# simonsobs/Pixell.jl

Hardware: AMD Instinct MI355X
Metric: Mpix/s CAR bilinear reproject (Float64) + % HBM roofline, 1/2/4/8 MI355X (higher is better)
Workload: dtype f64

## Files before the change

pixell.jl_amd/csrc/pxl_kernels.hip:

```cpp
#include <hip/hip_runtime.h>

#include <algorithm>
#include <mutex>
#include <vector>
#include <cmath>
#include <cstdarg>
#include <cstdio>
#include <cstring>
#include <new>
#include <type_traits>

#include "pxl_device.h"

using namespace pxl;

static thread_local char g_err[512] = "";

static int fail(int code, const char* fmt, ...) {
    va_list ap;
    va_start(ap, fmt);
    vsnprintf(g_err, sizeof(g_err), fmt, ap);
    va_end(ap);
    return code;
}
// ... 1131 lines not shown
int pxl_reproject_execute_f32(pxl_reproject_plan* pl, const float* src, float* dst, void* stream) {
    int rc = pxl_reproject_build_tables(pl, stream);
    if (rc) return rc;
    return pxl_reproject_execute_rows_f32(pl, src, dst, 0, pl->dst_nrows, stream);
}

int pxl_reproject_plan_src_rows(const pxl_reproject_plan* pl, int64_t* lo, int64_t* hi) {
    if (!pl || !lo || !hi) return fail(PXL_EINVAL, "plan_src_rows: null argument");
    int64_t l = INT64_MAX, h = INT64_MIN;
    for (int64_t r = 0; r < pl->dst_nrows; ++r) {
        int64_t j0 = pl->h_yj0[pl->dst_row0 + r];
        for (int64_t j = j0; j <= j0 + 1; ++j)
            if (j >= 1 && j <= pl->ny) { if (j - 1 < l) l = j - 1; if (j > h) h = j; }
    }
    if (l > h) { l = 0; h = 0; }
    *lo = l; *hi = h;
    return PXL_OK;
}

int pxl_reproject_plan_rows_covered(const pxl_reproject_plan* pl, int64_t have_lo, int64_t have_hi, int64_t* lo,
                                    int64_t* hi) {
    if (!pl || !lo || !hi) return fail(PXL_EINVAL, "plan_rows_covered: null argument");
    int64_t best_lo = 0, best_hi = 0, cur_lo = -1;
    for (int64_t r = 0; r <= pl->dst_nrows; ++r) {
        bool ok = false;
        if (r < pl->dst_nrows) {
            int64_t j0 = pl->h_yj0[pl->dst_row0 + r];
            ok = true;
            for (int64_t j = j0; j <= j0 + 1; ++j)
                if (j >= 1 && j <= pl->ny && !(j - 1 >= have_lo && j - 1 < have_hi)) ok = false;
        }
        if (ok) { if (cur_lo < 0) cur_lo = r; }
        else if (cur_lo >= 0) {
            if (r - cur_lo > best_hi - best_lo) { best_lo = cur_lo; best_hi = r; }
            cur_lo = -1;
        }
    }
    *lo = best_lo; *hi = best_hi;
    return PXL_OK;
}

int pxl_comm_unique_id(void* id128) {
    if (!id128) return fail(PXL_EINVAL, "comm_unique_id: null buffer (PXL_COMM_ID_BYTES bytes)");
    const RcclApi& nc = rccl_api(true);
    if (!nc.ok) return fail(PXL_ENODEV, "comm_unique_id: RCCL not available: %s", nc.where);
    static_assert(sizeof(ncclUniqueId) == PXL_COMM_ID_BYTES, "ncclUniqueId size");
    ncclUniqueId id;
    ncclResult_t r = nc.GetUniqueId(&id);
    if (r != ncclSuccess) return fail(PXL_EHIP, "comm_unique_id: ncclGetUniqueId: %s", nc.GetErrorString(r));
    memcpy(id128, &id, sizeof id);
    return PXL_OK;
}

int pxl_comm_init_rank(const void* id128, int rank, int nranks, void** comm) {
    if (!id128 || !comm) return fail(PXL_EINVAL, "comm_init_rank: null argument");
    *comm = nullptr;
    if (nranks < 1 || rank < 0 || rank >= nranks) return fail(PXL_EINVAL, "comm_init_rank: rank %d outside [0, %d)", rank, nranks);
    const RcclApi& nc = rccl_api(true);
    if (!nc.ok) return fail(PXL_ENODEV, "comm_init_rank: RCCL not available: %s", nc.where);
    ncclUniqueId id;
    memcpy(&id, id128, sizeof id);
    ncclComm_t c = nullptr;
    ncclResult_t r = nc.CommInitRank(&c, nranks, id, rank);
    if (r != ncclSuccess) return fail(PXL_EHIP, "comm_init_rank: ncclCommInitRank: %s", nc.GetErrorString(r));
    rccl_own_comm_add((void*)c);
    *comm = (void*)c;
    return PXL_OK;
}

int pxl_comm_destroy(void* comm) {
    if (!comm) return PXL_OK;
    if (!rccl_own_comm_erase(comm)) return fail(PXL_EINVAL, "comm_destroy: not a communicator created by pxl_comm_init_rank");
    const RcclApi& nc = rccl_api(false);
    if (!nc.ok) return fail(PXL_ENODEV, "comm_destroy: RCCL not available: %s", nc.where);
    ncclResult_t r = nc.CommDestroy((ncclComm_t)comm);
    if (r != ncclSuccess) return fail(PXL_EHIP, "comm_destroy: ncclCommDestroy: %s", nc.GetErrorString(r));
    return PXL_OK;
}

const char* pxl_comm_backend(void) {
    static thread_local char where[256];
    const RcclApi nc = rccl_api(false);
    snprintf(where, sizeof where, "%s", nc.where);
    return where;
}

int pxl_reproject_sharded_step_f64(pxl_reproject_plan* plan, double* src, double* dst, int64_t own_row0, int64_t own_nrows,
                                   const pxl_halo_xfer* sends, int nsends, const pxl_halo_xfer* recvs, int nrecvs,
                                   void* rccl_comm, void* stream) {
    return sharded_step_impl(plan, src, dst, own_row0, own_nrows, sends, nsends, recvs, nrecvs, rccl_comm, stream);
}

int pxl_reproject_sharded_step_f32(pxl_reproject_plan* plan, float* src, float* dst, int64_t own_row0, int64_t own_nrows,
                                   const pxl_halo_xfer* sends, int nsends, const pxl_halo_xfer* recvs, int nrecvs,
                                   void* rccl_comm, void* stream) {
    return sharded_step_impl(plan, src, dst, own_row0, own_nrows, sends, nsends, recvs, nrecvs, rccl_comm, stream);
}

int pxl_reproject_car_bilinear_f64(const pxl_car_wcs* wcs_in, const int64_t shape_in[3], const double* src,
                                   const pxl_car_wcs* wcs_out, const int64_t shape_out[2], double* dst,
                                   void* stream) {
    if (!shape_in || !shape_out) return fail(PXL_EINVAL, "reproject: null shape");
    pxl_reproject_plan* pl = nullptr;
    int rc = pxl_reproject_plan_create(wcs_in, shape_in, 0, shape_in[1], wcs_out, shape_out, 0, shape_out[1], &pl);
    if (rc) return rc;
    rc = pxl_reproject_execute(pl, src, dst, stream);
    if (rc == PXL_OK) {
        hipError_t e = hipStreamSynchronize((hipStream_t)stream);
        if (e != hipSuccess) rc = fail(PXL_EHIP, "reproject: %s", hipGetErrorString(e));
    }
    pxl_reproject_plan_destroy(pl);
    return rc;
}

int pxl_reproject_generic_last_tiles(int64_t* exact_tiles, int64_t* total_tiles, void* stream) {
    if (!exact_tiles || !total_tiles) return fail(PXL_EINVAL, "generic_last_tiles: null argument");
    int64_t total = 0;
    unsigned int* c = last_exact_word(-1, &total);
    if (!c) return fail(PXL_ENODEV, "generic_last_tiles: no counter on this device");
    unsigned int v = 0;
    HIP_TRY(hipMemcpyAsync(&v, c, 4, hipMemcpyDeviceToHost, (hipStream_t)stream));
    HIP_TRY(hipStreamSynchronize((hipStream_t)stream));
    *exact_tiles = v; *total_tiles = total;
    return PXL_OK;
}

struct pxl_generic_plan {
    GenericParams p;
    int64_t gx, gy, ntiles, exact;
    char* mem;
    LatticeWs ws;
    int device;
};

int pxl_generic_plan_create(const pxl_car_wcs* wcs_in, int proj_in, const int64_t shape_in[2],
                            const pxl_car_wcs* wcs_out, int proj_out, const int64_t shape_out[2],
                            void* stream, pxl_generic_plan** plan) {
    if (!plan) return fail(PXL_EINVAL, "generic_plan_create: null result");
    *plan = nullptr;
    GenericParams p;
    int rc = generic_params("generic_plan_create", wcs_in, proj_in, shape_in, wcs_out, proj_out, shape_out, &p);
    if (rc) return rc;
    const int64_t gx = (p.nxo + PXL_TW - 1) / PXL_TW, gy = (p.nyo + PXL_TH - 1) / PXL_TH;
    if (gy > 65535) return fail(PXL_EINVAL, "generic_plan_create: more than 65 535 tile rows (use the one-shot entry)");
    const int64_t ntiles = gx * gy;
    pxl_generic_plan* pl = new (std::nothrow) pxl_generic_plan();
    if (!pl) return fail(PXL_ENOMEM, "generic_plan_create: out of host memory");
    hipStream_t st = (hipStream_t)stream;
    hipError_t e = hipGetDevice(&pl->device);
    if (e == hipSuccess) e = hipMalloc((void**)&pl->mem, lattice_layout(nullptr, ntiles).bytes);
    if (e != hipSuccess) { (void)hipGetLastError(); delete pl; return fail(PXL_EHIP, "generic_plan_create: %s", hipGetErrorString(e)); }
    pl->ws = lattice_layout(pl->mem, ntiles);
    pl->gx = gx; pl->gy = gy; pl->ntiles = ntiles;
    p.exact_tiles = pl->ws.counter; p.exact_tiles_last = nullptr;
    pl->p = p;
    unsigned int host_count = 0;
    e = lattice_build(p, gx, ntiles, pl->ws, st);
    if (e == hipSuccess) e = hipGetLastError();
    if (e == hipSuccess) e = hipMemcpyAsync(&host_count, pl->ws.counter, 4, hipMemcpyDeviceToHost, st);
    if (e == hipSuccess) e = hipStreamSynchronize(st);
    if (e != hipSuccess) { (void)hipFree(pl->mem); delete pl; return fail(PXL_EHIP, "generic_plan_create: %s", hipGetErrorString(e)); }
    pl->exact = host_count;
    *plan = pl;
    return PXL_OK;
}

int pxl_generic_plan_execute(const pxl_generic_plan* plan, int64_t ncomp, const double* src, double* dst, void* stream) {
    if (!plan) return fail(PXL_EINVAL, "generic_plan_execute: null plan");
    if (ncomp < 1 || ncomp > 0x7fffffff) return fail(PXL_EINVAL, "generic_plan_execute: component count must be positive");
    if (!src || !dst) return fail(PXL_EINVAL, "generic_plan_execute: null src/dst");
    int dev = -1;
    if (hipGetDevice(&dev) != hipSuccess || dev != plan->device) return fail(PXL_EINVAL, "generic_plan_execute: plan belongs to device %d, current device is %d", plan->device, dev);
    GenericParams p = plan->p;
    p.src = src; p.dst = dst; p.nc = (int32_t)ncomp;
    hipStream_t st = (hipStream_t)stream;
    hipLaunchKernelGGL(k_reproject_generic_tiled3, dim3((unsigned)plan->gx, (unsigned)plan->gy), dim3(256), 0, st, p, (const double2*)plan->ws.lat, (const int32_t*)plan->ws.flag);
    if (plan->exact > 0)
        hipLaunchKernelGGL(k_reproject_generic_exact_tiles, dim3((unsigned)std::min<int64_t>(plan->ntiles, 256)), dim3(256), 0, st, p, (const int32_t*)plan->ws.flag, plan->gx, plan->ntiles);
    return check_launch("k_reproject_generic_tiled3 (plan)");
}

int pxl_generic_plan_tiles(const pxl_generic_plan* plan, int64_t* exact_tiles, int64_t* total_tiles) {
    if (!plan || !exact_tiles || !total_tiles) return fail(PXL_EINVAL, "generic_plan_tiles: null argument");
    *exact_tiles = plan->exact; *total_tiles = plan->ntiles;
    return PXL_OK;
}

int pxl_generic_plan_destroy(pxl_generic_plan* plan) {
    if (!plan) return PXL_OK;
    hipError_t e = plan->mem ? hipFree(plan->mem) : hipSuccess;
    delete plan;
    if (e != hipSuccess) return fail(PXL_EHIP, "generic_plan_destroy: %s", hipGetErrorString(e));
    return PXL_OK;
}

int pxl_reproject_generic_bilinear_f64(const pxl_car_wcs* wcs_in, int proj_in, const int64_t shape_in[3],
                                       const double* src, const pxl_car_wcs* wcs_out, int proj_out,
                                       const int64_t shape_out[2], double* dst, void* stream) {
    GenericParams p;
    int rcp = generic_params("reproject_generic", wcs_in, proj_in, shape_in, wcs_out, proj_out, shape_out, &p);
    if (rcp) return rcp;
    if (shape_in[2] < 1) return fail(PXL_EINVAL, "reproject_generic: shapes must be positive");
    if (!src || !dst) return fail(PXL_EINVAL, "reproject_generic: null src/dst");
    p.src = src; p.dst = dst; p.nc = (int32_t)shape_in[2];
    const int64_t gx = (p.nxo + PXL_TW - 1) / PXL_TW, gy = (p.nyo + PXL_TH - 1) / PXL_TH;
    if (env_int("PXL_GENERIC_EXACT", 0) || gy > 65535) {
        hipLaunchKernelGGL(k_reproject_generic, dim3(stream_grid(p.nxo * p.nyo, 256)), dim3(256), 0, (hipStream_t)stream, p);
        return check_launch("k_reproject_generic");
    }
    const int64_t ntiles = gx * gy;
    p.exact_tiles_last = last_exact_word(ntiles);
    hipStream_t st = (hipStream_t)stream;
    Scratch mem;
    if (int rc = mem.alloc(lattice_layout(nullptr, ntiles).bytes, st)) return rc;
    const LatticeWs ws = lattice_layout(mem.p, ntiles);
    p.exact_tiles = ws.counter;
    hipError_t me = lattice_build(p, gx, ntiles, ws, st);
    if (me != hipSuccess) {
        (void)hipGetLastError();
        return fail(PXL_EHIP, "reproject_generic: hipMemsetAsync: %s", hipGetErrorString(me));
    }
    hipLaunchKernelGGL(k_reproject_generic_tiled3, dim3((unsigned)gx, (unsigned)gy), dim3(256), 0, st, p, (const double2*)ws.lat, (const int32_t*)ws.flag);
    hipLaunchKernelGGL(k_reproject_generic_exact_tiles, dim3((unsigned)std::min<int64_t>(ntiles, 256)), dim3(256), 0, st, p, (const int32_t*)ws.flag, gx, ntiles);
    return mem.release("reproject_generic", check_launch("k_reproject_generic_tiled3"));
}

int pxl_sample_car_bilinear_f64(const pxl_car_wcs* wcs_in, const int64_t shape_in[3], const double* src,
                                int64_t src_row0, int64_t src_nrows, int64_t n, const double* sky, double* out,
                                void* stream) {
    return sample_impl(wcs_in, shape_in, src, src_row0, src_nrows, n, sky, out, stream);
}

int pxl_scatter_car_bilinear_f64(const pxl_car_wcs* wcs, const int64_t shape[3], double* dst, int64_t row0, int64_t nrows,
                                 int64_t n, const double* sky, const double* vals, void* stream) {
    PointCall c("scatter", wcs, shape, n, sky);
    if (int rc = check_points(c.rows(row0, nrows).reads(vals, 0).writes(dst, 0))) return rc;
    return launch_points(c, "k_scatter_bilinear", k_scatter_bilinear, PXL_SUNR, stream, dst, shape[0], shape[1], (int32_t)shape[2], row0, nrows,
                         car_periodic(wcs, shape[0]), n, (const double2*)sky, vals);
}

int pxl_sample_car_bilinear_f32(const pxl_car_wcs* wcs_in, const int64_t shape_in[3], const float* src,
                                int64_t src_row0, int64_t src_nrows, int64_t n, const double* sky, float* out,
                                void* stream) {
    return sample_impl(wcs_in, shape_in, src, src_row0, src_nrows, n, sky, out, stream);
}

int pxl_spline_prefilter_car_f64(const pxl_car_wcs* wcs, const int64_t shape[3], const double* src, double* coeffs, void* stream) {
    return spline_prefilter_impl<false>("spline_prefilter", wcs, shape, src, coeffs, stream);
}

int pxl_spline_prefilter_transpose_car_f64(const pxl_car_wcs* wcs, const int64_t shape[3], const double* src, double* dst, void* stream) {
    return spline_prefilter_impl<true>("spline_prefilter_transpose", wcs, shape, src, dst, stream);
}

int pxl_reproject_car_cubic_f64(const pxl_car_wcs* wcs_in, const int64_t shape_in[3], const double* coeffs,
                                const pxl_car_wcs* wcs_out, const int64_t shape_out[2], double* dst, void* stream) {
    if (!wcs_ok(wcs_in) || !wcs_ok(wcs_out)) return fail(PXL_EINVAL, "reproject_cubic: invalid WCS");
    if (int rc = spline_shape_check("reproject_cubic", shape_in)) return rc;
    if (!shape_out || shape_out[0] < 1 || shape_out[1] < 1) return fail(PXL_EINVAL, "reproject_cubic: output shape must be positive");
    if (shape_out[0] > 1000000000 || shape_out[1] > 65535LL * PXL_SPL_TH) return fail(PXL_EINVAL, "reproject_cubic: output axis too long");
    if (!coeffs || !dst) return fail(PXL_EINVAL, "reproject_cubic: null coefficients or output");
    const int64_t nx = shape_in[0], ny = shape_in[1], nc = shape_in[2], nxo = shape_out[0], nyo = shape_out[1];
    const uintptr_t cb = (uintptr_t)nx * (uintptr_t)ny * (uintptr_t)nc * 8, db = (uintptr_t)nxo * (uintptr_t)nyo * (uintptr_t)nc * 8;
    if (overlaps(coeffs, cb, dst, db)) return fail(PXL_EINVAL, "reproject_cubic: dst overlaps coeffs");
    hipStream_t st = (hipStream_t)stream;
    Scratch mem;
    if (int rc = mem.alloc(table_layout(nullptr, nxo, nyo).bytes, st)) return rc;
    const Tables t = table_layout(mem.p, nxo, nyo);
    SplineReproj p;
    p.coeffs = coeffs; p.dst = dst;
    p.xfx = t.xfx; p.yfy = t.yfy; p.xi0 = t.xi0; p.yj0 = t.yj0;
    p.nx = nx; p.ny = ny; p.nxo = nxo; p.nyo = nyo; p.periodic = car_periodic(wcs_in, nx);
    launch_build_tables(*wcs_in, nx, ny, *wcs_out, nxo, nyo, t, st);
    hipLaunchKernelGGL(k_reproject_cubic, dim3((unsigned)((nxo + 255) / 256), (unsigned)((nyo + PXL_SPL_TH - 1) / PXL_SPL_TH), (unsigned)nc),
                       dim3(256), 0, st, p);
    return mem.release("reproject_cubic", check_launch("k_reproject_cubic"));
}

int pxl_sample_car_cubic_f64(const pxl_car_wcs* wcs_in, const int64_t shape_in[3], const double* coeffs, int64_t n,
                             const double* sky, double* out, void* stream) {
    PointCall c("sample_cubic", wcs_in, shape_in, n, sky);
    if (int rc = check_points(c.cubic_coeffs(coeffs).needs(out))) return rc;
    return launch_points(c, "k_sample_cubic", k_sample_cubic, 1, stream, coeffs, shape_in[0], shape_in[1], (int32_t)shape_in[2],
                         car_periodic(wcs_in, shape_in[0]), n, (const double2*)sky, out);
}

int pxl_scatter_car_cubic_f64(const pxl_car_wcs* wcs, const int64_t shape[3], double* dst, int64_t n, const double* sky,
                              const double* vals, void* stream) {
    PointCall c("scatter_cubic", wcs, shape, n, sky);
    if (int rc = check_points(c.cubic_map().reads(vals, 0).writes(dst, 0))) return rc;
    return launch_points(c, "k_scatter_cubic", k_scatter_cubic, PXL_CUNR, stream, dst, shape[0], shape[1], (int32_t)shape[2],
                         car_periodic(wcs, shape[0]), n, (const double2*)sky, vals);
}

int pxl_sample_car_pol_bilinear_f64(const pxl_car_wcs* wcs_in, const int64_t shape_in[3], const double* src, int64_t src_row0,
                                    int64_t src_nrows, int64_t n, const double* sky, const double* resp, double* out, void* stream) {
    PointCall c("sample_pol", wcs_in, shape_in, n, sky);
    if (int rc = check_points(c.rows(src_row0, src_nrows).polarised(resp).map(src).needs(out))) return rc;
    return launch_points(c, "k_sample_pol_bilinear", k_sample_pol_bilinear, PXL_PSUNR, stream, src, shape_in[0], shape_in[1], src_row0, src_nrows,
                         car_periodic(wcs_in, shape_in[0]), n, (const double2*)sky, (const double2*)resp, out);
}

int pxl_sample_car_pol_cubic_f64(const pxl_car_wcs* wcs_in, const int64_t shape_in[3], const double* coeffs, int64_t n,
                                 const double* sky, const double* resp, double* out, void* stream) {
    PointCall c("sample_pol_cubic", wcs_in, shape_in, n, sky);
    if (int rc = check_points(c.cubic_coeffs(coeffs).polarised(resp).needs(out))) return rc;
    return launch_points(c, "k_sample_pol_cubic", k_sample_pol_cubic, 1, stream, coeffs, shape_in[0], shape_in[1],
                         car_periodic(wcs_in, shape_in[0]), n, (const double2*)sky, (const double2*)resp, out);
}

int pxl_scatter_car_pol_bilinear_f64(const pxl_car_wcs* wcs, const int64_t shape[3], double* dst, int64_t row0, int64_t nrows, int64_t n,
                                     const double* sky, const double* resp, const double* vals, int mode, void* stream) {
    PointCall c("scatter_pol", wcs, shape, n, sky);
    if (int rc = check_points(c.rows(row0, nrows).polarised(resp, mode).reads(vals, 1).writes(dst, mode ? 6 : 3))) return rc;
    return launch_points(c, "k_scatter_pol_bilinear", mode ? k_scatter_pol_bilinear<6> : k_scatter_pol_bilinear<3>, PXL_SUNR, stream, dst,
                         shape[0], shape[1], row0, nrows, car_periodic(wcs, shape[0]), n, (const double2*)sky, (const double2*)resp, vals);
}

int pxl_scatter_car_pol_cubic_f64(const pxl_car_wcs* wcs, const int64_t shape[3], double* dst, int64_t n, const double* sky,
                                  const double* resp, const double* vals, int mode, void* stream) {
    PointCall c("scatter_pol_cubic", wcs, shape, n, sky);
    if (int rc = check_points(c.cubic_map().polarised(resp, mode).reads(vals, 1).writes(dst, mode ? 6 : 3))) return rc;
    return launch_points(c, "k_scatter_pol_cubic", mode ? k_scatter_pol_cubic<6> : k_scatter_pol_cubic<3>, PXL_CUNR, stream, dst, shape[0],
                         shape[1], car_periodic(wcs, shape[0]), n, (const double2*)sky, (const double2*)resp, vals);
}

int pxl_normal_car_pol_bilinear_f64(const pxl_car_wcs* wcs, const int64_t shape[3], const double* x3, double* y3, int64_t n,
                                    const double* sky, const double* resp, const double* w, void* stream) {
    PointCall c("normal_pol", wcs, shape, n, sky);
    if (int rc = check_points(c.polarised(resp).map(x3).reads(w, 1).writes(y3, 3))) return rc;
    const uintptr_t mb = c.idle ? 0 : (uintptr_t)(3 * shape[1] * shape[0]) * 8;
    if (overlaps(y3, mb, x3, mb)) return fail(PXL_EINVAL, "normal_pol: y overlaps x");
    return launch_points(c, "k_normal_pol_bilinear", k_normal_pol_bilinear, PXL_NUNR, stream, x3, y3, shape[0], shape[1],
                         car_periodic(wcs, shape[0]), n, (const double2*)sky, (const double2*)resp, w);
}

int pxl_sample_car_nearest_f64(const pxl_car_wcs* wcs_in, const int64_t shape_in[3], const double* src, int64_t src_row0,
                               int64_t src_nrows, int64_t n, const double* sky, double* out, void* stream) {
    PointCall c("sample_nearest", wcs_in, shape_in, n, sky);
    if (int rc = check_points(c.rows(src_row0, src_nrows).map(src).needs(out))) return rc;
    return launch_points(c, "k_sample_nearest", k_sample_nearest, PXL_ZUNR, stream, src, shape_in[0], shape_in[1], (int32_t)shape_in[2], src_row0,
                         src_nrows, car_periodic(wcs_in, shape_in[0]), n, (const double2*)sky, out);
}

int pxl_scatter_car_nearest_f64(const pxl_car_wcs* wcs, const int64_t shape[3], double* dst, int64_t row0, int64_t nrows,
                                int64_t n, const double* sky, const double* vals, void* stream) {
    PointCall c("scatter_nearest", wcs, shape, n, sky);
    if (int rc = check_points(c.rows(row0, nrows).reads(vals, 0).writes(dst, 0))) return rc;
    return launch_points(c, "k_scatter_nearest", k_scatter_nearest, PXL_ZUNR, stream, dst, shape[0], shape[1], (int32_t)shape[2], row0, nrows,
                         car_periodic(wcs, shape[0]), n, (const double2*)sky, vals);
}

int pxl_sample_car_pol_nearest_f64(const pxl_car_wcs* wcs_in, const int64_t shape_in[3], const double* src, int64_t src_row0,
                                   int64_t src_nrows, int64_t n, const double* sky, const double* resp, double* out, void* stream) {
    PointCall c("sample_pol_nearest", wcs_in, shape_in, n, sky);
    if (int rc = check_points(c.rows(src_row0, src_nrows).polarised(resp).map(src).needs(out))) return rc;
    return launch_points(c, "k_sample_pol_nearest", k_sample_pol_nearest, PXL_ZUNR, stream, src, shape_in[0], shape_in[1], src_row0, src_nrows,
                         car_periodic(wcs_in, shape_in[0]), n, (const double2*)sky, (const double2*)resp, out);
}

int pxl_scatter_car_pol_nearest_f64(const pxl_car_wcs* wcs, const int64_t shape[3], double* dst, int64_t row0, int64_t nrows, int64_t n,
                                    const double* sky, const double* resp, const double* vals, int mode, void* stream) {
    PointCall c("scatter_pol_nearest", wcs, shape, n, sky);
    if (int rc = check_points(c.rows(row0, nrows).polarised(resp, mode).reads(vals, 1).writes(dst, mode ? 6 : 3))) return rc;
    return launch_points(c, "k_scatter_pol_nearest", mode ? k_scatter_pol_nearest<6> : k_scatter_pol_nearest<3>, PXL_ZUNR, stream, dst,
                         shape[0], shape[1], row0, nrows, car_periodic(wcs, shape[0]), n, (const double2*)sky, (const double2*)resp, vals);
}

int pxl_bin_car_pol_nearest_f64(const pxl_car_wcs* wcs, const int64_t shape[3], double* rhs3, double* weights6, int64_t n,
                                const double* sky, const double* resp, const double* d, const double* w, void* stream) {
    PointCall c("bin_pol_nearest", wcs, shape, n, sky);
    if (int rc = check_points(c.polarised(resp).reads(d, 1).reads(w, 1).writes(rhs3, 3).writes(weights6, 6))) return rc;
    const uintptr_t pb = c.idle ? 0 : (uintptr_t)(shape[1] * shape[0]) * 8;
    if (overlaps(rhs3, 3 * pb, weights6, 6 * pb)) return fail(PXL_EINVAL, "bin_pol_nearest: rhs3 overlaps weights6");
    return launch_points(c, "k_bin_pol_nearest", k_bin_pol_nearest, PXL_ZUNR, stream, rhs3, weights6, shape[0], shape[1],
                         car_periodic(wcs, shape[0]), n, (const double2*)sky, (const double2*)resp, d, w);
}
// ... 367 lines not shown
```

pixell.jl_amd/csrc/pxl_sample.h:

```cpp
#pragma once

struct GenericParams {
    const double* src; double* dst;
    int64_t nx, ny, nxo, nyo;
    int32_t nc, periodic, proj_in, proj_out;
    CarAffine out_car; TanParams out_tan;
    Sky2Pix in_car; TanParams in_tan;
    unsigned int* exact_tiles;
    unsigned int* exact_tiles_last;
};
__device__ inline void generic_coords(const GenericParams& p, double i, double j, double* x, double* y, bool* visible) {
    double ra, dec;
    if (p.proj_out == PXL_PROJ_TAN) tan_pix2sky(p.out_tan, i, j, &ra, &dec);
    else { ra = p2s_ra(p.out_car, i); dec = p2s_dec(p.out_car, j); }
    *visible = true;
    if (p.proj_in == PXL_PROJ_TAN) {
        tan_sky2pix(p.in_tan, ra, dec, x, y);
        *visible = (p.in_tan.sd0 * sin(dec) + cos(dec) * cos(ra - p.in_tan.a0) * p.in_tan.cd0) > 0.0;
    } else { *x = s2p_x(p.in_car, ra); *y = s2p_y(p.in_car, dec); }
}
__device__ inline void generic_store(const GenericParams& p, int64_t t, double x, double y, bool visible) {
    const int64_t total = p.nxo * p.nyo;
    const bool fin = isfinite(x) && isfinite(y);
    int32_t i0, j0; double fx, fy;
    split_cell(x, &i0, &fx);
    split_cell(y, &j0, &fy);
    const bool jin = j0 >= 1 && j0 < p.ny;
    const bool iin = p.periodic ? (i0 >= 0 && i0 <= p.nx) : (i0 >= 1 && i0 < p.nx);
    if (visible && fin && jin && iin) {
        const int64_t ia = (i0 >= 1 ? i0 : p.nx) - 1, ib = (i0 < p.nx ? i0 + 1 : 1) - 1;
        const int64_t ra = (int64_t)(j0 - 1) * p.nx, rb = ra + p.nx;
        for (int c = 0; c < p.nc; ++c) {
            const double* pl = p.src + (int64_t)c * p.nx * p.ny;
            const double top = (1 - fx) * pl[ra + ia] + fx * pl[ra + ib];
            const double bot = (1 - fx) * pl[rb + ia] + fx * pl[rb + ib];
            p.dst[(int64_t)c * total + t] = (1 - fy) * top + fy * bot;
        }
        return;
    }
    for (int c = 0; c < p.nc; ++c) {
        SrcView m{p.src + (int64_t)c * p.nx * p.ny, p.nx, p.ny, 0, p.ny, p.periodic};
        double v = visible ? bilerp_cells(m, i0, fx, j0, fy) : 0.0;
        p.dst[(int64_t)c * total + t] = fin ? v : __builtin_nan("");
    }
}
__global__ __launch_bounds__(256) void k_reproject_generic(GenericParams p) {
    const int64_t total = p.nxo * p.nyo;
    int64_t stride = (int64_t)gridDim.x * blockDim.x;
    for (int64_t t = (int64_t)blockIdx.x * blockDim.x + threadIdx.x; t < total; t += stride) {
        const int64_t jr = t / p.nxo, i = t - jr * p.nxo;
        double x, y; bool visible;
        generic_coords(p, (double)(i + 1), (double)(jr + 1), &x, &y, &visible);
        generic_store(p, t, x, y, visible);
    }
}

#define PXL_TILED_TOL 1e-10
#ifndef PXL_TNX
#define PXL_TNX 7
#endif
#ifndef PXL_TNY
#define PXL_TNY 6
#endif
#define PXL_TCHK0 (PXL_TNX * PXL_TNY <= 40 ? 40 : 48)
#define PXL_TNCHK 12
#ifndef PXL_TH
#define PXL_TH 32
#endif
#ifndef PXL_TW
#define PXL_TW 128
#endif
#define PXL_TROWS (256 / PXL_TW)
template <int N>
__device__ inline void lagrange_weights(double u, double h, double* w) {
    double d[N];
#pragma unroll
    for (int c = 0; c < N; ++c) d[c] = u - c * h;
    double hp = 1.0;
#pragma unroll
    for (int c = 1; c < N; ++c) hp *= h;
    const double rh = 1.0 / hp;
#pragma unroll
    for (int a = 0; a < N; ++a) {
        double num = 1.0;
        int k = 1;
#pragma unroll
        for (int c = 0; c < N; ++c)
            if (c != a) { num *= d[c]; k *= (a - c); }
        w[a] = num * (rh / (double)k);
    }
}
struct TileWeights { double wx[PXL_TW][PXL_TNX]; double wy[PXL_TH][PXL_TNY]; };
constexpr double lag_w(int n, double h, double u, int a) {
    double num = 1.0, den = 1.0;
    for (int c = 0; c < n; ++c)
        if (c != a) { num *= (u - c * h); den *= ((a - c) * h); }
    return num / den;
}
constexpr TileWeights make_tile_weights() {
    TileWeights t{};
    for (int u = 0; u < PXL_TW; ++u)
        for (int a = 0; a < PXL_TNX; ++a) t.wx[u][a] = lag_w(PXL_TNX, (PXL_TW - 1.0) / (PXL_TNX - 1), (double)u, a);
    for (int v = 0; v < PXL_TH; ++v)
        for (int b = 0; b < PXL_TNY; ++b) t.wy[v][b] = lag_w(PXL_TNY, (PXL_TH - 1.0) / (PXL_TNY - 1), (double)v, b);
    return t;
}
__constant__ TileWeights c_tile_weights = make_tile_weights();

__global__ __launch_bounds__(256) void k_generic_lattice(GenericParams p, int64_t ntx, int64_t ntiles,
                                                         double2* __restrict__ lat, int32_t* __restrict__ flag) {
    __shared__ double lx[4][PXL_TNX * PXL_TNY], ly[4][PXL_TNX * PXL_TNY];
    __shared__ int bad[4];
    const int w = threadIdx.x >> 6, k = threadIdx.x & 63;
    const int64_t tile = (int64_t)blockIdx.x * 4 + w;
    const bool live = tile < ntiles;
    const int64_t ti0 = live ? (tile % ntx) * PXL_TW : 0, tj0 = live ? (tile / ntx) * PXL_TH : 0;
    const double hx = (PXL_TW - 1.0) / (PXL_TNX - 1), hy = (PXL_TH - 1.0) / (PXL_TNY - 1);
    if (k == 0) bad[w] = 0;
    __syncthreads();
    double ex = 0.0, ey = 0.0, cu = 0.0, cv = 0.0;
    bool is_check = false;
    if (live && k < PXL_TNX * PXL_TNY) {
        const int a = k % PXL_TNX, b = k / PXL_TNX;
        bool vis;
        generic_coords(p, (double)(ti0 + 1) + a * hx, (double)(tj0 + 1) + b * hy, &ex, &ey, &vis);
        lx[w][k] = ex; ly[w][k] = ey;
        lat[tile * (PXL_TNX * PXL_TNY) + k] = make_double2(ex, ey);
        if (!vis || !isfinite(ex) || !isfinite(ey)) bad[w] = 1;
    } else if (live && k >= PXL_TCHK0 && k < PXL_TCHK0 + PXL_TNCHK) {
        const double uf[12] = {0.10, 0.50, 0.90, 0.30, 0.70, 0.95, 0.04, 0.21, 0.41, 0.59, 0.79, 0.985};
        const double vf[12] = {0.12, 0.47, 0.82, 0.70, 0.23, 0.94, 0.55, 0.97, 0.05, 0.88, 0.35, 0.63};
        const double us[12] = {uf[0] * (PXL_TW - 1), uf[1] * (PXL_TW - 1), uf[2] * (PXL_TW - 1), uf[3] * (PXL_TW - 1), uf[4] * (PXL_TW - 1),
                               uf[5] * (PXL_TW - 1), uf[6] * (PXL_TW - 1), uf[7] * (PXL_TW - 1), uf[8] * (PXL_TW - 1), uf[9] * (PXL_TW - 1),
                               uf[10] * (PXL_TW - 1), uf[11] * (PXL_TW - 1)};
        const double vs[12] = {vf[0] * (PXL_TH - 1), vf[1] * (PXL_TH - 1), vf[2] * (PXL_TH - 1), vf[3] * (PXL_TH - 1), vf[4] * (PXL_TH - 1),
                               vf[5] * (PXL_TH - 1), vf[6] * (PXL_TH - 1), vf[7] * (PXL_TH - 1), vf[8] * (PXL_TH - 1), vf[9] * (PXL_TH - 1),
                               vf[10] * (PXL_TH - 1), vf[11] * (PXL_TH - 1)};
        cu = us[k - PXL_TCHK0]; cv = vs[k - PXL_TCHK0];
        bool vis;
        generic_coords(p, (double)(ti0 + 1) + cu, (double)(tj0 + 1) + cv, &ex, &ey, &vis);
        is_check = true;
        if (!vis || !isfinite(ex) || !isfinite(ey)) bad[w] = 1;
    }
    __syncthreads();
    if (is_check && !bad[w]) {
        double wx[PXL_TNX], wy[PXL_TNY];
        lagrange_weights<PXL_TNX>(cu, hx, wx);
        lagrange_weights<PXL_TNY>(cv, hy, wy);
        double sx = 0.0, sy = 0.0;
        for (int b = 0; b < PXL_TNY; ++b)
            for (int a = 0; a < PXL_TNX; ++a) {
                const double ww = wx[a] * wy[b];
                sx = __builtin_fma(ww, lx[w][b * PXL_TNX + a], sx);
                sy = __builtin_fma(ww, ly[w][b * PXL_TNX + a], sy);
            }
        if (!(fabs(sx - ex) <= PXL_TILED_TOL && fabs(sy - ey) <= PXL_TILED_TOL)) bad[w] = 1;
    }
    __syncthreads();
    if (live && k == 0) {
        flag[tile] = bad[w];
        if (bad[w] && p.exact_tiles) atomicAdd(p.exact_tiles, 1u);
    }
}
__global__ __launch_bounds__(256) void k_reproject_generic_exact_tiles(GenericParams p, const int32_t* __restrict__ flag, int64_t gx, int64_t ntiles) {
    const unsigned int counted = p.exact_tiles ? *p.exact_tiles : 1u;
    if (blockIdx.x == 0 && threadIdx.x == 0 && p.exact_tiles && p.exact_tiles_last) *p.exact_tiles_last = counted;
    if (counted == 0u) return;
    for (int64_t tile = blockIdx.x; tile < ntiles; tile += gridDim.x) {
        if (!flag[tile]) continue;
        const int64_t bx = tile % gx, by = tile / gx;
        const int64_t i = bx * PXL_TW + (threadIdx.x & (PXL_TW - 1)), jr0 = by * PXL_TH + threadIdx.x / PXL_TW;
        if (i >= p.nxo) continue;
        for (int q = 0; q < PXL_TH / PXL_TROWS; ++q) {
            const int64_t jr = jr0 + PXL_TROWS * q;
            if (jr < p.nyo) {
                double x, y; bool visible;
                generic_coords(p, (double)(i + 1), (double)(jr + 1), &x, &y, &visible);
                generic_store(p, jr * p.nxo + i, x, y, visible);
            }
        }
    }
}
__global__ __launch_bounds__(256) void k_reproject_generic_tiled3(GenericParams p, const double2* __restrict__ lat,
                                                                  const int32_t* __restrict__ flag) {
    const int64_t tile = (int64_t)blockIdx.y * gridDim.x + blockIdx.x;
    const int64_t ti0 = (int64_t)blockIdx.x * PXL_TW, tj0 = (int64_t)blockIdx.y * PXL_TH;
    const int tid = threadIdx.x;
    const int cx = tid & (PXL_TW - 1), ry = __builtin_amdgcn_readfirstlane(tid / PXL_TW);
    const int64_t i = ti0 + cx;
    if (i >= p.nxo) return;
    if (flag[tile]) return;
    const double2* L = lat + tile * (PXL_TNX * PXL_TNY);
    double wx[PXL_TNX];
#pragma unroll
    for (int a = 0; a < PXL_TNX; ++a) wx[a] = c_tile_weights.wx[cx][a];
    double colx[PXL_TNY], coly[PXL_TNY];
#pragma unroll
    for (int b = 0; b < PXL_TNY; ++b) {
        double sx = 0.0, sy = 0.0;
#pragma unroll
        for (int a = 0; a < PXL_TNX; ++a) { const double2 v = L[b * PXL_TNX + a]; sx = __builtin_fma(wx[a], v.x, sx); sy = __builtin_fma(wx[a], v.y, sy); }
        colx[b] = sx; coly[b] = sy;
    }
    auto coords = [&](int r, double* x, double* y) {
        double sx = 0.0, sy = 0.0;
#pragma unroll
        for (int b = 0; b < PXL_TNY; ++b) { const double wy = c_tile_weights.wy[r][b]; sx = __builtin_fma(wy, colx[b], sx); sy = __builtin_fma(wy, coly[b], sy); }
        *x = sx; *y = sy;
    };
    const int64_t total = p.nxo * p.nyo;
    const uint32_t nxm1 = (uint32_t)(p.nx - 1), nym1 = (uint32_t)(p.ny - 1);
    const int32_t nx32 = (int32_t)p.nx;
    const bool small = p.nx * p.ny < 0x7fffffffLL && p.nx < 0x7fffffffLL;
    struct __attribute__((packed, aligned(8))) Pair { double a, b; };
    uint32_t slow_rows = 0;
    constexpr int NQ = PXL_TH / PXL_TROWS;
#ifndef PXL_T3_G
#define PXL_T3_G 4
#endif

    constexpr int G = PXL_T3_G;
#pragma unroll
    for (int q0 = 0; q0 < NQ; q0 += G) {
        double fx[G], fy[G];
        int64_t off[G];
        bool ok = true;
#pragma unroll
        for (int g = 0; g < G; ++g) {
            const int r = ry + PXL_TROWS * (q0 + g);
            double x, y;
            coords(r, &x, &y);
            const double flx = floor(x), fly = floor(y);
            fx[g] = x - flx; fy[g] = y - fly;
            const int32_t i0 = (int32_t)flx, j0 = (int32_t)fly;
            ok = ok && (uint32_t)(i0 - 1) < nxm1 && (uint32_t)(j0 - 1) < nym1;
            off[g] = small ? (int64_t)((j0 - 1) * nx32 + (i0 - 1)) : (int64_t)(j0 - 1) * p.nx + (i0 - 1);
        }
        const bool inside = tj0 + ry + PXL_TROWS * (q0 + G - 1) < p.nyo;
        if (inside && __all(ok)) {
            for (int c = 0; c < p.nc; ++c) {
                const double* pl = p.src + (int64_t)c * p.nx * p.ny;
                Pair tp[G], bt[G];
#pragma unroll
                for (int g = 0; g < G; ++g) { tp[g] = *reinterpret_cast<const Pair*>(pl + off[g]); bt[g] = *reinterpret_cast<const Pair*>(pl + off[g] + p.nx); }
#pragma unroll
                for (int g = 0; g < G; ++g) {
                    const double top = (1 - fx[g]) * tp[g].a + fx[g] * tp[g].b;
                    const double bot = (1 - fx[g]) * bt[g].a + fx[g] * bt[g].b;
                    __builtin_nontemporal_store((1 - fy[g]) * top + fy[g] * bot, &p.dst[(int64_t)c * total + (tj0 + ry + PXL_TROWS * (q0 + g)) * p.nxo + i]);
                }
            }
        } else {
#pragma unroll
            for (int g = 0; g < G; ++g)
                if (tj0 + ry + PXL_TROWS * (q0 + g) < p.nyo) slow_rows |= 1u << (q0 + g);
        }
    }
#pragma unroll 1
    while (slow_rows) {
        const int q = __builtin_ctz(slow_rows);
        slow_rows &= slow_rows - 1;
        const int r = ry + PXL_TROWS * q;
        double x, y;
        double sx = 0.0, sy = 0.0;
#pragma unroll
        for (int b = 0; b < PXL_TNY; ++b) { const double wy = c_tile_weights.wy[r][b]; sx = __builtin_fma(wy, colx[b], sx); sy = __builtin_fma(wy, coly[b], sy); }
        x = sx; y = sy;
        generic_store(p, (tj0 + r) * p.nxo + i, x, y, true);
    }
}

__device__ __noinline__ double2 sample_coords_slow(double a, double d, double ia0, double a0, double rda, double px, double cx,
                                                   double rpx, double id0, double d0, double rdd, double py, double cy, double rpy) {
    return make_double2(rewind(ia0 + (a - a0) * rda, px, cx, rpx), rewind(id0 + (d - d0) * rdd, py, cy, rpy));
}
__device__ inline void sample_coords(const Sky2Pix& s, double a, double d, double* x, double* y) {
    if (s.safe && s.form != PXL_FORM_DIV) {
        bool ok0, ok1;
        *x = rewind_try(s.c.ia0 + (a - s.c.a0) * s.rda, s.px, s.cx, s.rpx, &ok0);
        *y = rewind_try(s.c.id0 + (d - s.c.d0) * s.rdd, s.py, s.cy, s.rpy, &ok1);
        if (__builtin_expect(!(ok0 && ok1), 0)) {
            const double2 r = sample_coords_slow(a, d, s.c.ia0, s.c.a0, s.rda, s.px, s.cx, s.rpx, s.c.id0, s.c.d0, s.rdd, s.py, s.cy, s.rpy);
            *x = r.x; *y = r.y;
        }
        return;
    }
    *x = s2p_x(s, a); *y = s2p_y(s, d);
}
template <typename T>
__global__ __launch_bounds__(256) void k_sample_bilinear(Sky2Pix s, const T* __restrict__ src, int64_t nx,
                                                         int64_t ny, int32_t nc, int64_t row0, int64_t nrows,
                                                         int periodic, int64_t n, const double2* __restrict__ sky,
                                                         T* __restrict__ out) {
    const int64_t plane = nx * nrows;
    for (Trip<PXL_SUNR> trip; trip.k0 < n; trip.next()) {
        double2 ad[PXL_SUNR];
        trip.load(sky, n, ad, make_double2(0.0, 0.0));
        Cell2 cell[PXL_SUNR];
#pragma unroll
        for (int u = 0; u < PXL_SUNR; ++u) cell[u] = cell2<false>(s, ad[u], nx, ny, row0, nrows, periodic, true);
        for (int c = 0; c < nc; ++c) {
            const T* pl = src + (int64_t)c * plane;
            Taps2 m[PXL_SUNR];
#pragma unroll
            for (int u = 0; u < PXL_SUNR; ++u) m[u] = gather2_wide(pl, cell[u], sky);
#pragma unroll
            for (int u = 0; u < PXL_SUNR; ++u)
                if (__builtin_expect(!cell[u].wide, 0)) gather2_fixup(pl, cell[u], m[u]);
#pragma unroll
            for (int u = 0; u < PXL_SUNR; ++u) {
                const double v = lerp2(m[u], cell[u].fx, cell[u].fy);
                if (trip.k(u) < n) out[(int64_t)c * n + trip.k(u)] = (T)(cell[u].fin ? v : __builtin_nan(""));
            }
        }
    }
}

template <typename T> struct Vec2T;
template <> struct Vec2T<double> { typedef double2 type; };
template <> struct Vec2T<float>  { typedef float2 type; };

template <typename T> struct PairGroup {
    static constexpr int E = 64 / (2 * (int)sizeof(T));
    static constexpr int C = E - 1;
    __host__ __device__ static inline int64_t groups(int64_t nx) { return (nx + C - 1) / C; }
};
template <typename T>
__global__ __launch_bounds__(256) void k_build_rowpairs(const T* __restrict__ src, int64_t nx, int64_t nrows,
                                                        typename Vec2T<T>::type* __restrict__ pairs, int fronts) {
    typedef typename Vec2T<T>::type T2;
    constexpr int E = PairGroup<T>::E, C = PairGroup<T>::C;
    const int64_t pitch = PairGroup<T>::groups(nx) * E;
    const int64_t t = (int64_t)blockIdx.x * blockDim.x + threadIdx.x;
    if (t >= pitch) return;
    const int64_t g = t / E, e = t - g * E;
    int64_t i = g * C + e;
    if (i >= nx) i %= nx;
    const int64_t c = blockIdx.z;
    const T* pl = src + c * nx * nrows;
    T2* out = pairs + c * pitch * (nrows + 1);
    const int64_t per = (gridDim.y + fronts - 1) / fronts;
    const int64_t yy = fronts > 1 ? (int64_t)(blockIdx.y % fronts) * per + blockIdx.y / fronts : (int64_t)blockIdx.y;
    const int64_t p0 = yy * PXL_POS_ROWS;
    if (p0 > nrows) return;
    const int64_t p1 = (p0 + PXL_POS_ROWS <= nrows) ? p0 + PXL_POS_ROWS : nrows + 1;
    T above = (p0 >= 1) ? pl[(p0 - 1) * nx + i] : (T)0;
    for (int64_t p = p0; p < p1; ++p) {
        const T here = (p < nrows) ? pl[p * nx + i] : (T)0;
        T2 v; v.x = above; v.y = here;
        out[p * pitch + t] = v;
        above = here;
    }
}

template <typename T> struct PairsUnroll { static constexpr int value = PXL_SUNR; };
template <typename T>
__global__ __launch_bounds__(256) void k_sample_pairs(Sky2Pix s, const typename Vec2T<T>::type* __restrict__ pairs,
                                                      int64_t nx, int64_t ny, int32_t nc, int64_t row0, int64_t nrows,
                                                      int periodic, int64_t n, const double2* __restrict__ sky,
                                                      T* __restrict__ out) {
    typedef typename Vec2T<T>::type T2;
    constexpr int SUNR = PairsUnroll<T>::value;
    constexpr int E = PairGroup<T>::E, C = PairGroup<T>::C;
    const int64_t pitch = PairGroup<T>::groups(nx) * E;
    const int64_t plane = pitch * (nrows + 1);
    for (Trip<SUNR> trip; trip.k0 < n; trip.next()) {
        double2 ad[SUNR];
        trip.load(sky, n, ad, make_double2(0.0, 0.0));
        int64_t oa[SUNR], ob[SUNR];
        double fx[SUNR], fy[SUNR];
        bool fin[SUNR];
#pragma unroll
        for (int u = 0; u < SUNR; ++u) {
            double x, y;
            sample_coords(s, ad[u].x, ad[u].y, &x, &y);
            fin[u] = isfinite(x) && isfinite(y);
            int32_t i0, j0;
            split_cell(x, &i0, &fx[u]);
            split_cell(y, &j0, &fy[u]);
            int64_t ia = i0, ib = (int64_t)i0 + 1;
            bool oka = true, okb = true;
            if (periodic) { ia = wrap_col(ia, nx); ib = wrap_col(ib, nx); }
            else { oka = (ia >= 1 && ia <= nx); okb = (ib >= 1 && ib <= nx); }
            const int64_t p = (int64_t)j0 - row0;
            const bool rows = (p >= 0 && p <= nrows);
            const uint32_t ca = (uint32_t)((oka ? ia : ib) - 1), ga = ca / (uint32_t)C;
            const int64_t ent = p * pitch + (int64_t)ga * E + (ca - ga * (uint32_t)C);
            oa[u] = (rows && oka) ? ent : -1;
            ob[u] = (rows && okb) ? (oka ? ent + 1 : ent) : -1;
        }
        for (int c = 0; c < nc; ++c) {
            const T2* pl = pairs + (int64_t)c * plane;
            T2 a[SUNR], b[SUNR];
#pragma unroll
            for (int u = 0; u < SUNR; ++u) {
                a[u] = pl[oa[u] >= 0 ? oa[u] : 0];
                b[u] = pl[ob[u] >= 0 ? ob[u] : 0];
            }
#pragma unroll
            for (int u = 0; u < SUNR; ++u) {
                if (oa[u] < 0) { a[u].x = (T)0; a[u].y = (T)0; }
                if (ob[u] < 0) { b[u].x = (T)0; b[u].y = (T)0; }
            }
#pragma unroll
            for (int u = 0; u < SUNR; ++u) {
                double top = (1 - fx[u]) * (double)a[u].x + fx[u] * (double)b[u].x;
                double bot = (1 - fx[u]) * (double)a[u].y + fx[u] * (double)b[u].y;
                double v = (1 - fy[u]) * top + fy[u] * bot;
                if (trip.k(u) < n) out[(int64_t)c * n + trip.k(u)] = (T)(fin[u] ? v : __builtin_nan(""));
            }
        }
    }
}
```

Baseline: 391,100.

## Fuse lattice build, tiled interpolation and exact fallback into one kernel

The one-shot generic reproject path now launches a single fused kernel per tile. One wavefront computes the interpolation lattice and check points into shared memory and validates them with wave-level votes, then the whole block either interpolates from the lattice or falls back to exact per-pixel coordinates. This removes the scratch allocation, the global lattice and flag round-trip, and two extra kernel launches. In exchange, three of four waves sit idle during lattice construction, and the kernel now carries a launch-bounds occupancy hint.

```diff
diff --git a/pixell.jl_amd/csrc/pxl_kernels.hip b/pixell.jl_amd/csrc/pxl_kernels.hip
--- a/pixell.jl_amd/csrc/pxl_kernels.hip
+++ b/pixell.jl_amd/csrc/pxl_kernels.hip
@@ -1307,7 +1307,7 @@
     if (e != hipSuccess) { (void)hipGetLastError(); delete pl; return fail(PXL_EHIP, "generic_plan_create: %s", hipGetErrorString(e)); }
     pl->ws = lattice_layout(pl->mem, ntiles);
     pl->gx = gx; pl->gy = gy; pl->ntiles = ntiles;
-    p.exact_tiles = pl->ws.counter; p.exact_tiles_last = nullptr;
+    p.exact_tiles = pl->ws.counter;
     pl->p = p;
     unsigned int host_count = 0;
     e = lattice_build(p, gx, ntiles, pl->ws, st);
@@ -1363,21 +1363,17 @@
         hipLaunchKernelGGL(k_reproject_generic, dim3(stream_grid(p.nxo * p.nyo, 256)), dim3(256), 0, (hipStream_t)stream, p);
         return check_launch("k_reproject_generic");
     }
-    const int64_t ntiles = gx * gy;
-    p.exact_tiles_last = last_exact_word(ntiles);
+    p.exact_tiles = last_exact_word(gx * gy);
     hipStream_t st = (hipStream_t)stream;
-    Scratch mem;
-    if (int rc = mem.alloc(lattice_layout(nullptr, ntiles).bytes, st)) return rc;
-    const LatticeWs ws = lattice_layout(mem.p, ntiles);
-    p.exact_tiles = ws.counter;
-    hipError_t me = lattice_build(p, gx, ntiles, ws, st);
-    if (me != hipSuccess) {
-        (void)hipGetLastError();
-        return fail(PXL_EHIP, "reproject_generic: hipMemsetAsync: %s", hipGetErrorString(me));
-    }
-    hipLaunchKernelGGL(k_reproject_generic_tiled3, dim3((unsigned)gx, (unsigned)gy), dim3(256), 0, st, p, (const double2*)ws.lat, (const int32_t*)ws.flag);
-    hipLaunchKernelGGL(k_reproject_generic_exact_tiles, dim3((unsigned)std::min<int64_t>(ntiles, 256)), dim3(256), 0, st, p, (const int32_t*)ws.flag, gx, ntiles);
-    return mem.release("reproject_generic", check_launch("k_reproject_generic_tiled3"));
+    if (p.exact_tiles) {
+        hipError_t me = hipMemsetAsync(p.exact_tiles, 0, 4, st);
+        if (me != hipSuccess) {
+            (void)hipGetLastError();
+            return fail(PXL_EHIP, "reproject_generic: hipMemsetAsync: %s", hipGetErrorString(me));
+        }
+    }
+    hipLaunchKernelGGL(k_reproject_generic_fused, dim3((unsigned)gx, (unsigned)gy), dim3(256), 0, st, p);
+    return check_launch("k_reproject_generic_fused");
 }
 
 int pxl_sample_car_bilinear_f64(const pxl_car_wcs* wcs_in, const int64_t shape_in[3], const double* src,
diff --git a/pixell.jl_amd/csrc/pxl_sample.h b/pixell.jl_amd/csrc/pxl_sample.h
--- a/pixell.jl_amd/csrc/pxl_sample.h
+++ b/pixell.jl_amd/csrc/pxl_sample.h
@@ -7,7 +7,6 @@
     CarAffine out_car; TanParams out_tan;
     Sky2Pix in_car; TanParams in_tan;
     unsigned int* exact_tiles;
-    unsigned int* exact_tiles_last;
 };
 __device__ inline void generic_coords(const GenericParams& p, double i, double j, double* x, double* y, bool* visible) {
     double ra, dec;
@@ -107,26 +106,16 @@
 }
 __constant__ TileWeights c_tile_weights = make_tile_weights();
 
-__global__ __launch_bounds__(256) void k_generic_lattice(GenericParams p, int64_t ntx, int64_t ntiles,
-                                                         double2* __restrict__ lat, int32_t* __restrict__ flag) {
-    __shared__ double lx[4][PXL_TNX * PXL_TNY], ly[4][PXL_TNX * PXL_TNY];
-    __shared__ int bad[4];
-    const int w = threadIdx.x >> 6, k = threadIdx.x & 63;
-    const int64_t tile = (int64_t)blockIdx.x * 4 + w;
-    const bool live = tile < ntiles;
-    const int64_t ti0 = live ? (tile % ntx) * PXL_TW : 0, tj0 = live ? (tile / ntx) * PXL_TH : 0;
+struct LatticePoint { double ex, ey, cu, cv; bool is_node, is_check, bad; };
+__device__ inline LatticePoint lattice_point(const GenericParams& p, int64_t ti0, int64_t tj0, int k, bool live) {
     const double hx = (PXL_TW - 1.0) / (PXL_TNX - 1), hy = (PXL_TH - 1.0) / (PXL_TNY - 1);
-    if (k == 0) bad[w] = 0;
-    __syncthreads();
-    double ex = 0.0, ey = 0.0, cu = 0.0, cv = 0.0;
-    bool is_check = false;
+    LatticePoint q{0.0, 0.0, 0.0, 0.0, false, false, false};
     if (live && k < PXL_TNX * PXL_TNY) {
         const int a = k % PXL_TNX, b = k / PXL_TNX;
         bool vis;
-        generic_coords(p, (double)(ti0 + 1) + a * hx, (double)(tj0 + 1) + b * hy, &ex, &ey, &vis);
-        lx[w][k] = ex; ly[w][k] = ey;
-        lat[tile * (PXL_TNX * PXL_TNY) + k] = make_double2(ex, ey);
-        if (!vis || !isfinite(ex) || !isfinite(ey)) bad[w] = 1;
+        generic_coords(p, (double)(ti0 + 1) + a * hx, (double)(tj0 + 1) + b * hy, &q.ex, &q.ey, &vis);
+        q.is_node = true;
+        q.bad = !vis || !isfinite(q.ex) || !isfinite(q.ey);
     } else if (live && k >= PXL_TCHK0 && k < PXL_TCHK0 + PXL_TNCHK) {
         const double uf[12] = {0.10, 0.50, 0.90, 0.30, 0.70, 0.95, 0.04, 0.21, 0.41, 0.59, 0.79, 0.985};
         const double vf[12] = {0.12, 0.47, 0.82, 0.70, 0.23, 0.94, 0.55, 0.97, 0.05, 0.88, 0.35, 0.63};
@@ -136,61 +125,76 @@
         const double vs[12] = {vf[0] * (PXL_TH - 1), vf[1] * (PXL_TH - 1), vf[2] * (PXL_TH - 1), vf[3] * (PXL_TH - 1), vf[4] * (PXL_TH - 1),
                                vf[5] * (PXL_TH - 1), vf[6] * (PXL_TH - 1), vf[7] * (PXL_TH - 1), vf[8] * (PXL_TH - 1), vf[9] * (PXL_TH - 1),
                                vf[10] * (PXL_TH - 1), vf[11] * (PXL_TH - 1)};
-        cu = us[k - PXL_TCHK0]; cv = vs[k - PXL_TCHK0];
+        q.cu = us[k - PXL_TCHK0]; q.cv = vs[k - PXL_TCHK0];
         bool vis;
-        generic_coords(p, (double)(ti0 + 1) + cu, (double)(tj0 + 1) + cv, &ex, &ey, &vis);
-        is_check = true;
-        if (!vis || !isfinite(ex) || !isfinite(ey)) bad[w] = 1;
-    }
+        generic_coords(p, (double)(ti0 + 1) + q.cu, (double)(tj0 + 1) + q.cv, &q.ex, &q.ey, &vis);
+        q.is_check = true;
+        q.bad = !vis || !isfinite(q.ex) || !isfinite(q.ey);
+    }
+    return q;
+}
+__device__ inline bool lattice_check_fails(const LatticePoint& q, const double2* L) {
+    const double hx = (PXL_TW - 1.0) / (PXL_TNX - 1), hy = (PXL_TH - 1.0) / (PXL_TNY - 1);
+    double wx[PXL_TNX], wy[PXL_TNY];
+    lagrange_weights<PXL_TNX>(q.cu, hx, wx);
+    lagrange_weights<PXL_TNY>(q.cv, hy, wy);
+    double sx = 0.0, sy = 0.0;
+    for (int b = 0; b < PXL_TNY; ++b)
+        for (int a = 0; a < PXL_TNX; ++a) {
+            const double ww = wx[a] * wy[b];
+            sx = __builtin_fma(ww, L[b * PXL_TNX + a].x, sx);
+            sy = __builtin_fma(ww, L[b * PXL_TNX + a].y, sy);
+        }
+    return !(fabs(sx - q.ex) <= PXL_TILED_TOL && fabs(sy - q.ey) <= PXL_TILED_TOL);
+}
+
+__global__ __launch_bounds__(256) void k_generic_lattice(GenericParams p, int64_t ntx, int64_t ntiles,
+                                                         double2* __restrict__ lat, int32_t* __restrict__ flag) {
+    __shared__ double2 lxy[4][PXL_TNX * PXL_TNY];
+    __shared__ int bad[4];
+    const int w = threadIdx.x >> 6, k = threadIdx.x & 63;
+    const int64_t tile = (int64_t)blockIdx.x * 4 + w;
+    const bool live = tile < ntiles;
+    const int64_t ti0 = live ? (tile % ntx) * PXL_TW : 0, tj0 = live ? (tile / ntx) * PXL_TH : 0;
+    if (k == 0) bad[w] = 0;
     __syncthreads();
-    if (is_check && !bad[w]) {
-        double wx[PXL_TNX], wy[PXL_TNY];
-        lagrange_weights<PXL_TNX>(cu, hx, wx);
-        lagrange_weights<PXL_TNY>(cv, hy, wy);
-        double sx = 0.0, sy = 0.0;
-        for (int b = 0; b < PXL_TNY; ++b)
-            for (int a = 0; a < PXL_TNX; ++a) {
-                const double ww = wx[a] * wy[b];
-                sx = __builtin_fma(ww, lx[w][b * PXL_TNX + a], sx);
-                sy = __builtin_fma(ww, ly[w][b * PXL_TNX + a], sy);
-            }
-        if (!(fabs(sx - ex) <= PXL_TILED_TOL && fabs(sy - ey) <= PXL_TILED_TOL)) bad[w] = 1;
-    }
+    const LatticePoint q = lattice_point(p, ti0, tj0, k, live);
+    if (q.is_node) {
+        lxy[w][k] = make_double2(q.ex, q.ey);
+        lat[tile * (PXL_TNX * PXL_TNY) + k] = make_double2(q.ex, q.ey);
+    }
+    if (q.bad) bad[w] = 1;
+    __syncthreads();
+    if (q.is_check && !bad[w] && lattice_check_fails(q, lxy[w])) bad[w] = 1;
     __syncthreads();
     if (live && k == 0) {
         flag[tile] = bad[w];
         if (bad[w] && p.exact_tiles) atomicAdd(p.exact_tiles, 1u);
     }
 }
+__device__ inline void generic_tile_exact(const GenericParams& p, int64_t bx, int64_t by) {
+    const int64_t i = bx * PXL_TW + (threadIdx.x & (PXL_TW - 1)), jr0 = by * PXL_TH + threadIdx.x / PXL_TW;
+    if (i >= p.nxo) return;
+    for (int q = 0; q < PXL_TH / PXL_TROWS; ++q) {
+        const int64_t jr = jr0 + PXL_TROWS * q;
+        if (jr < p.nyo) {
+            double x, y; bool visible;
+            generic_coords(p, (double)(i + 1), (double)(jr + 1), &x, &y, &visible);
+            generic_store(p, jr * p.nxo + i, x, y, visible);
+        }
+    }
+}
 __global__ __launch_bounds__(256) void k_reproject_generic_exact_tiles(GenericParams p, const int32_t* __restrict__ flag, int64_t gx, int64_t ntiles) {
-    const unsigned int counted = p.exact_tiles ? *p.exact_tiles : 1u;
-    if (blockIdx.x == 0 && threadIdx.x == 0 && p.exact_tiles && p.exact_tiles_last) *p.exact_tiles_last = counted;
-    if (counted == 0u) return;
-    for (int64_t tile = blockIdx.x; tile < ntiles; tile += gridDim.x) {
-        if (!flag[tile]) continue;
-        const int64_t bx = tile % gx, by = tile / gx;
-        const int64_t i = bx * PXL_TW + (threadIdx.x & (PXL_TW - 1)), jr0 = by * PXL_TH + threadIdx.x / PXL_TW;
-        if (i >= p.nxo) continue;
-        for (int q = 0; q < PXL_TH / PXL_TROWS; ++q) {
-            const int64_t jr = jr0 + PXL_TROWS * q;
-            if (jr < p.nyo) {
-                double x, y; bool visible;
-                generic_coords(p, (double)(i + 1), (double)(jr + 1), &x, &y, &visible);
-                generic_store(p, jr * p.nxo + i, x, y, visible);
-            }
-        }
-    }
-}
-__global__ __launch_bounds__(256) void k_reproject_generic_tiled3(GenericParams p, const double2* __restrict__ lat,
-                                                                  const int32_t* __restrict__ flag) {
-    const int64_t tile = (int64_t)blockIdx.y * gridDim.x + blockIdx.x;
+    if (p.exact_tiles && *p.exact_tiles == 0u) return;
+    for (int64_t tile = blockIdx.x; tile < ntiles; tile += gridDim.x)
+        if (flag[tile]) generic_tile_exact(p, tile % gx, tile / gx);
+}
+__device__ __forceinline__ void generic_tile_pixels(const GenericParams& p, const double2* __restrict__ L) {
     const int64_t ti0 = (int64_t)blockIdx.x * PXL_TW, tj0 = (int64_t)blockIdx.y * PXL_TH;
     const int tid = threadIdx.x;
     const int cx = tid & (PXL_TW - 1), ry = __builtin_amdgcn_readfirstlane(tid / PXL_TW);
     const int64_t i = ti0 + cx;
     if (i >= p.nxo) return;
-    if (flag[tile]) return;
-    const double2* L = lat + tile * (PXL_TNX * PXL_TNY);
     double wx[PXL_TNX];
 #pragma unroll
     for (int a = 0; a < PXL_TNX; ++a) wx[a] = c_tile_weights.wx[cx][a];
@@ -268,6 +272,33 @@
         x = sx; y = sy;
         generic_store(p, (tj0 + r) * p.nxo + i, x, y, true);
     }
+}
+__global__ __launch_bounds__(256) void k_reproject_generic_tiled3(GenericParams p, const double2* __restrict__ lat,
+                                                                  const int32_t* __restrict__ flag) {
+    const int64_t tile = (int64_t)blockIdx.y * gridDim.x + blockIdx.x;
+    if (flag[tile]) return;
+    generic_tile_pixels(p, lat + tile * (PXL_TNX * PXL_TNY));
+}
+__global__ __launch_bounds__(256, 4) void k_reproject_generic_fused(GenericParams p) {
+    __shared__ double2 L[PXL_TNX * PXL_TNY];
+    __shared__ int s_bad;
+    const int64_t tile = (int64_t)blockIdx.y * gridDim.x + blockIdx.x;
+    const int w = __builtin_amdgcn_readfirstlane((int)(threadIdx.x >> 6)), k = threadIdx.x & 63;
+    if (w == (int)(tile & 3)) {
+        const LatticePoint q = lattice_point(p, (int64_t)blockIdx.x * PXL_TW, (int64_t)blockIdx.y * PXL_TH, k, true);
+        if (q.is_node) L[k] = make_double2(q.ex, q.ey);
+        bool bad = __any(q.bad);
+        __builtin_amdgcn_s_waitcnt(0xc07f);
+        __builtin_amdgcn_wave_barrier();
+        if (!bad) bad = __any(q.is_check && lattice_check_fails(q, L));
+        if (k == 0) {
+            s_bad = bad;
+            if (bad && p.exact_tiles) atomicAdd(p.exact_tiles, 1u);
+        }
+    }
+    __syncthreads();
+    if (__builtin_amdgcn_readfirstlane(s_bad)) generic_tile_exact(p, blockIdx.x, blockIdx.y);
+    else generic_tile_pixels(p, L);
 }
 
 __device__ __noinline__ double2 sample_coords_slow(double a, double d, double ia0, double a0, double rda, double px, double cx,
```

Measured after the change: 389,100. No clear change (-0.5%).
